# bliunlpr/Robust_e2e_gan

Measured on AMD Instinct MI355X. Metric: joint_train utterances/sec, higher is better.
Workload: dtype f32; 1 GPU; config4: joint_train.py full GAN+ASR step, B=32 per GPU, T=800, F=257->80, L=40, V=4233, enhancer 2xBLSTM-256, VGG+3xBLSTMP-512, loc-attention decoder 300, D basic ndf64, Adadelta; global_batch=32, per_rank_batch=32, parallelism=dp1, utterance_lengths=560..800 frames (mean 680 of T=800)

## Files before the change

robust_e2e_gan_amd/csrc/common.h:

```cpp
#pragma once
#include <hip/hip_runtime.h>
#include <mutex>
#include <stdint.h>
#include <stdlib.h>
#include <stdio.h>
#include <string.h>

#include "../../include/re2e.h"

typedef float f32x4 __attribute__((ext_vector_type(4)));
typedef float f32x16 __attribute__((ext_vector_type(16)));

#define RE2E_WAVE 64

void re2e_set_error(const char* fmt, ...);
bool re2e_stream_is_filler(hipStream_t stream);

#define RE2E_CHECK_ARG(cond, msg)                     \
  do {                                                \
    if (!(cond)) {                                    \
      re2e_set_error("%s: %s", __func__, msg);        \
      return RE2E_EINVAL;                             \
    }                                                 \
  } while (0)

#define RE2E_LAUNCH_CHECK()                                                        \
  do {                                                                             \
    hipError_t e__ = hipGetLastError();                                            \
    if (e__ != hipSuccess) {                                                       \
      re2e_set_error("%s: launch failed: %s", __func__, hipGetErrorString(e__));   \
      return RE2E_EHIP;                                                            \
    }                                                                              \
  } while (0)

#ifdef RE2E_EXPERIMENTS
static inline const char* exp_env(const char* name) { return getenv(name); }
#else
static inline const char* exp_env(const char*) { return nullptr; }
#endif

struct LdsLimit {
  std::mutex m;
  size_t set = 0;
  void ensure(const void* fn, size_t bytes) {
    std::lock_guard<std::mutex> g(m);
    if (bytes > set) {
      (void)hipFuncSetAttribute(fn, hipFuncAttributeMaxDynamicSharedMemorySize, (int)bytes);
      set = bytes;
    }
  }
};

static inline int cdiv(long a, long b) { return (int)((a + b - 1) / b); }

__device__ __forceinline__ float sigmoidf_(float x) { return 1.0f / (1.0f + __expf(-x)); }
__device__ __forceinline__ float tanhf_(float x) {
  float ax = fabsf(x);
  float e = __expf(-2.0f * ax);
  float t = (1.0f - e) / (1.0f + e);
  return copysignf(t, x);
}

__device__ __forceinline__ float wave_sum(float v) {
#pragma unroll
  for (int o = 32; o > 0; o >>= 1) v += __shfl_xor(v, o, 64);
  return v;
}
__device__ __forceinline__ float wave_max(float v) {
#pragma unroll
  for (int o = 32; o > 0; o >>= 1) v = fmaxf(v, __shfl_xor(v, o, 64));
  return v;
}

__device__ __forceinline__ float block_sum(float v, float* red) {
  v = wave_sum(v);
  int w = threadIdx.x >> 6, l = threadIdx.x & 63;
  __syncthreads();
  if (l == 0) red[w] = v;
  __syncthreads();
  int nw = (blockDim.x + 63) >> 6;
  float r = 0.f;
  for (int i = 0; i < nw; ++i) r += red[i];
  return r;
}
__device__ __forceinline__ float block_max(float v, float* red) {
  v = wave_max(v);
  int w = threadIdx.x >> 6, l = threadIdx.x & 63;
  __syncthreads();
  if (l == 0) red[w] = v;
  __syncthreads();
  int nw = (blockDim.x + 63) >> 6;
  float r = -3.0e38f;
  for (int i = 0; i < nw; ++i) r = fmaxf(r, red[i]);
  return r;
}

__device__ __forceinline__ float apply_act(float v, int act) {
  switch (act) {
    case RE2E_ACT_TANH: return tanhf_(v);
    case RE2E_ACT_RELU: return fmaxf(v, 0.f);
    case RE2E_ACT_LRELU: return v > 0.f ? v : 0.2f * v;
    case RE2E_ACT_SIGMOID: return sigmoidf_(v);
    default: return v;
  }
}

struct ConvGeom {
  const float* in; int NI, H, W, C; int PH, PW; int KH, KW; int SY, SX, DY, DX, OY0, OX0;
};

struct OutMap {
  float* out; long ldc; int remap; int PH, PW, OHF, OWF, osy, osx, ooy, oox;
  __device__ long off(int row) const {
    if (!remap) return (long)row * ldc;
    int j = row % PW; int t = row / PW; int i = t % PH; int n = t / PH;
    return (((long)n * OHF + i * osy + ooy) * OWF + j * osx + oox) * ldc;
  }
};

bool thin_conv_forward(const ConvGeom& g, const float* wg, int Cout, const OutMap& o, const float* bias, int act,
                       float beta, hipStream_t st);
int thin_wgrad_slabs(int C, int Cout, int KH, int KW, long P, long rows);
void thin_wgrad(const ConvGeom& g, const float* dout, int Cout, float* slabs, int nslab, hipStream_t st);

int gemm_kslices_tn(int M, int N, int K, int ns, const float* A, long lda, const float* B, long ldb, float* out, hipStream_t st, int nolog = 0);
int gemm_kslices(int M, int N, int K, int ns, const float* A, long lda, const float* B, long ldb, float* out, hipStream_t st, int nolog = 0);
size_t gemm_nt2_workspace_bytes(int M, int N, int K);
int gemm_nt2(int M, int N, int K, const float* A, long lda, const float* B, long ldb, float* C, long ldc, const float* bias, const float* bias2,
             int act, float beta, const float* mul, float* mask_out, const int* lens, int T, void* ws, size_t wsb, hipStream_t st,
             const int* rowmap = nullptr, int phys_rows = 0, int ident_rows = 0);
int gemm_nt2_kslices(int M, int N, int Ks, int ns, const float* A, long lda, const float* B, long ldb, float* out, hipStream_t st, int nolog);
size_t gemm_tn2_workspace_bytes(int M, int N, int K);
int gemm_tn2(int M, int N, int K, const float* A, long lda, const float* B, long ldb, float* C, long ldc, const float* bias, const float* bias2,
             int act, float beta, void* ws, size_t wsb, hipStream_t st);
int conv_nt2(const ConvGeom& g, int M, const float* wg, int Cout, float* out, long ldc, const float* bias, int act, float beta, int ncls,
             const int* cls_oy0, const int* cls_ox0, long cls_wstride, int remap, int OHF, int OWF, int osy, int osx, const int* ooy, const int* oox,
             hipStream_t st);
bool halo_conv3x3(const ConvGeom& g, const float* wg, int Cout, float* out, const float* bias, int act, float beta, const float* mask,
                  hipStream_t st, float* pool_out = nullptr, unsigned char* pool_idx = nullptr);
```

robust_e2e_gan_amd/csrc/core.hip:

```cpp
#include <stdarg.h>

#include <mutex>

#include "common.h"

static thread_local char g_err[512] = "";

void re2e_set_error(const char* fmt, ...) {
  va_list ap;
  va_start(ap, fmt);
  vsnprintf(g_err, sizeof(g_err), fmt, ap);
  va_end(ap);
}

extern "C" int re2e_version(void) { return RE2E_ABI_VERSION; }

extern "C" const char* re2e_last_error(void) { return g_err; }

extern "C" int re2e_device_ok(void) {
  hipDeviceProp_t prop;
  hipError_t e = hipGetDeviceProperties(&prop, 0);
  if (e != hipSuccess) {
    re2e_set_error("re2e_device_ok: %s", hipGetErrorString(e));
    return RE2E_EHIP;
  }
  return strncmp(prop.gcnArchName, "gfx950", 6) == 0 ? 1 : 0;
}

namespace {
std::mutex g_role_mu;
hipStream_t g_filler[64];
int g_nfiller = 0;
}

extern "C" int re2e_stream_role(hipStream_t stream, int role) {
  RE2E_CHECK_ARG(role == RE2E_STREAM_DEFAULT || role == RE2E_STREAM_FILLER, "role must be RE2E_STREAM_DEFAULT or RE2E_STREAM_FILLER");
  std::lock_guard<std::mutex> lock(g_role_mu);
  int at = -1;
  for (int i = 0; i < g_nfiller; ++i) if (g_filler[i] == stream) at = i;
  if (role == RE2E_STREAM_FILLER) {
    if (at >= 0) return RE2E_OK;
    if (g_nfiller == 64) { re2e_set_error("re2e_stream_role: more than 64 filler streams"); return RE2E_EINVAL; }
    g_filler[g_nfiller++] = stream;
  } else if (at >= 0) {
    g_filler[at] = g_filler[--g_nfiller];
  }
  return RE2E_OK;
}

bool re2e_stream_is_filler(hipStream_t stream) {
  static const bool ignore = exp_env("RE2E_IGNORE_STREAM_ROLE") != nullptr;
  if (ignore) return false;
  std::lock_guard<std::mutex> lock(g_role_mu);
  for (int i = 0; i < g_nfiller; ++i) if (g_filler[i] == stream) return true;
  return false;
}
```

robust_e2e_gan_amd/csrc/gemm_nt.hip:

```cpp
#include <stdlib.h>

#include "common.h"

namespace {

typedef unsigned u32x4_t __attribute__((ext_vector_type(4)));
constexpr unsigned OOB = 0x80000000u;

template <int WM_, int WN_, int TM_, int TN_, int BK_, int ST_, int WPS_>
struct NtCfg {
  static constexpr int WM = WM_, WN = WN_, TM = TM_, TN = TN_, BK = BK_, ST = ST_, WPS = WPS_;
  static constexpr int BM = WM_ * TM_ * 32, BN = WN_ * TN_ * 32;
  static constexpr int NW = WM_ * WN_, THREADS = NW * 64;
  static constexpr int RPP = 256 / BK_;
  static constexpr int CPR = BK_ / 4;
  static constexpr int RPL = 64 / BK_;
  static constexpr int PA = BM / RPP, PB = BN / RPP;
  static constexpr int NPW = (PA + PB) / NW;
  static constexpr int NPA = PA / NW;
  static constexpr int STAGE = (BM + BN) * BK_;
  static constexpr int NQ = BK_ / 8;
  static constexpr size_t LDS_BYTES = (size_t)ST_ * STAGE * 4;
  static_assert(PA % NW == 0 && PB % NW == 0, "pieces must divide over the waves per operand");
  static_assert(BK_ == 16 || BK_ == 32 || BK_ == 64, "BK");
// ... 320 lines not shown
            const unsigned soff = (unsigned)rowq * (unsigned)p.ldc * 4u;
            const unsigned vo = (rows_in || rowq + TM * 4 * lh < p.M) ? vlane : OOB;
            fTN v;
#pragma unroll
            for (int b = 0; b < TN; ++b) v[b] = apply_act(acc[a][b][r] + bq[b], act);
            if constexpr (TN == 4) {
              if (acc_old) v += __builtin_bit_cast(fTN, __builtin_amdgcn_raw_buffer_load_b128(rsC, vo, soff, 0));
              __builtin_amdgcn_raw_buffer_store_b128(__builtin_bit_cast(u32x4_t, v), rsC, vo, soff, 0);
            } else {
              typedef unsigned u32x2_t __attribute__((ext_vector_type(2)));
              if (acc_old) v += __builtin_bit_cast(fTN, __builtin_amdgcn_raw_buffer_load_b64(rsC, vo, soff, 0));
              __builtin_amdgcn_raw_buffer_store_b64(__builtin_bit_cast(u32x2_t, v), rsC, vo, soff, 0);
            }
          }
      }
    } else
    if (finish) {
      const __amdgpu_buffer_rsrc_t rsC = __builtin_amdgcn_make_buffer_rsrc(p.C + (MODE == 0 ? cls * p.batch_c : 0L), 0, 0x7FFFFFF0u, 0x00020000);
      const unsigned vlane = ((unsigned)(TNF ? TM * lr : lr) * (unsigned)p.ldc + 4u * (unsigned)lh) * 4u;
      const bool interior = !CONV && m0 + BM <= p.M && n0 + BN <= p.N;
      unsigned vrow[TM];
      const bool mapped = MODE == 0 && p.rowmap != nullptr && m0 + BM > p.ident_rows;
      if constexpr (MODE == 0) {
        if (mapped) {
#pragma unroll
          for (int a = 0; a < TM; ++a) {
            const int row = m0 + (wm * TM + a) * 32 + lr;
            vrow[a] = row < p.M ? (unsigned)(((long)p.rowmap[row] * p.ldc + 4 * lh) * 4) : OOB;
          }
        }
      }
      if constexpr (CONV) {
#pragma unroll
        for (int a = 0; a < TM; ++a) {
          const int row = m0 + (wm * TM + a) * 32 + lr;
          bool ok = row < p.M;
          long off = (long)row * p.ldc;
          if (p.remap) {
            const int px = row % p.cPW, t2 = row / p.cPW, py = t2 % p.cPH, n = t2 / p.cPH;
            const int oy = py * p.osy + p.ooy[cls], ox = px * p.osx + p.oox[cls];
            ok = ok && oy < p.OHF && ox < p.OWF;
            off = (((long)n * p.OHF + oy) * p.OWF + ox) * p.ldc;
          }
          vrow[a] = ok ? (unsigned)((off + 4 * lh) * 4) : OOB;
        }
      }
      const bool has_bias = p.bias != nullptr, has_bias2 = p.bias2 != nullptr;
      const int act = p.act;
      const bool acc_old = p.beta != 0.f;
#pragma unroll
      for (int b = 0; b < TN; ++b)
#pragma unroll
        for (int g = 0; g < 4; ++g) {
          const int colq = n0 + (wn * TN + b) * 32 + 8 * g;
          f32x4 bq = {0.f, 0.f, 0.f, 0.f};
          const bool col_ok = colq + 4 * lh < p.N;
          if (has_bias && col_ok) bq += *reinterpret_cast<const f32x4*>(p.bias + colq + 4 * lh);
          if (has_bias2 && col_ok) bq += *reinterpret_cast<const f32x4*>(p.bias2 + colq + 4 * lh);
#pragma unroll
          for (int a = 0; a < TM; ++a) {
            const int rowq = TNF ? m0 + wm * TM * 32 + a : m0 + (wm * TM + a) * 32;
            unsigned soff = ((unsigned)rowq * (unsigned)p.ldc + (unsigned)colq) * 4u;
            unsigned vo = (interior || (col_ok && rowq + (TNF ? TM * lr : lr) < p.M)) ? vlane : OOB;
            if constexpr (CONV) { soff = (unsigned)colq * 4u; vo = col_ok ? vrow[a] : OOB; }
            if constexpr (MODE == 0) { if (mapped) { soff = (unsigned)colq * 4u; vo = col_ok ? vrow[a] : OOB; } }
            f32x4 v = {acc[a][b][4 * g], acc[a][b][4 * g + 1], acc[a][b][4 * g + 2], acc[a][b][4 * g + 3]};
            v += bq;
            if (act == RE2E_ACT_TANH) {
#pragma unroll
              for (int e = 0; e < 4; ++e) v[e] = tanhf_(v[e]);
            } else if (act == RE2E_ACT_SIGMOID) {
#pragma unroll
              for (int e = 0; e < 4; ++e) v[e] = sigmoidf_(v[e]);
            } else if (act == RE2E_ACT_RELU) {
#pragma unroll
              for (int e = 0; e < 4; ++e) v[e] = v[e] < 0.f ? 0.f : v[e];
            } else if (act == RE2E_ACT_LRELU) {
#pragma unroll
              for (int e = 0; e < 4; ++e) v[e] = v[e] < 0.f ? 0.2f * v[e] : v[e];
            }
            if (acc_old) v += __builtin_bit_cast(f32x4, __builtin_amdgcn_raw_buffer_load_b128(rsC, vo, soff, 0));
            __builtin_amdgcn_raw_buffer_store_b128(__builtin_bit_cast(u32x4_t, v), rsC, vo, soff, 0);
          }
        }
    }
    u0 += ke - kb;
  }
}

using N256x128k32s3 = NtCfg<4, 2, 2, 2, 32, 3, 2>;
using N256x128k16s3 = NtCfg<4, 2, 2, 2, 16, 3, 4>;
using N128x128k32s2 = NtCfg<2, 2, 2, 2, 32, 2, 2>;
using N128x128k16s3 = NtCfg<2, 2, 2, 2, 16, 3, 3>;
using N128x64k16s4 = NtCfg<2, 2, 2, 1, 16, 4, 3>;
using N256x64k16s3 = NtCfg<4, 1, 2, 2, 16, 3, 2>;
using T128x128k16s3 = NtCfg<2, 2, 2, 2, 16, 3, 3>;

struct NtVariant { int id, bm, bn, bk, wg_per_cu; double tflops; };
const NtVariant VARIANTS[] = {{1, 256, 128, 32, 1, 130.0}, {3, 256, 128, 16, 2, 138.0}, {5, 128, 128, 32, 2, 130.0},
                              {6, 128, 128, 16, 3, 137.0}, {8, 128, 64, 16, 3, 136.0},  {9, 256, 64, 16, 2, 128.0}};

struct NtPlan { int variant; int wg_per_cu; int bm, bn, bk; int ntm, ntn, nkt, n_dp, g_sk; size_t bytes; double est; };

inline int num_cus() {
  static const int cus = [] { int dev = 0, n = 256; if (hipGetDevice(&dev) == hipSuccess) (void)hipDeviceGetAttribute(&n, hipDeviceAttributeMultiprocessorCount, dev); return n; }();
  return cus;
}

NtPlan nt2_plan_variant(const NtVariant& v, int M, int N, int K, int sk) {
  NtPlan pl;
  memset(&pl, 0, sizeof(pl));
  pl.variant = v.id; pl.bm = v.bm; pl.bn = v.bn; pl.bk = v.bk; pl.wg_per_cu = v.wg_per_cu;
  pl.ntm = cdiv(M, pl.bm); pl.ntn = cdiv(N, pl.bn); pl.nkt = cdiv(K, pl.bk);
  const long T = (long)pl.ntm * pl.ntn, cus = num_cus();
  const long R = T % cus;
  const double slab = (double)v.bm * v.bn * 4.0;
  const double t_tile = 2.0 * v.bm * v.bn * (double)K / (v.tflops * 1e12 / cus);
  const double t_over = 1.0e-6 + slab / 25e9;
  pl.n_dp = (int)T; pl.g_sk = 0;
  pl.est = (double)cdiv(T, cus) * (t_tile + t_over);
  if (sk && R != 0) {
    const long U = R * pl.nkt;
    long g = cus;
    if (T == R && v.bm * v.bn <= 128 * 256) { const char* e = exp_env("RE2E_NT2_TAILWG"); g = cus * (e ? atoi(e) : 1); }
    const long min_units = 128 / pl.bk;
    if (U / g < min_units) g = U / min_units;
    if (g >= 8) g &= ~7L;
    const double parts = (double)g / (double)R + 1.0;
    const double t_fix = (7e-6 + (double)g * slab / 2.4e12) * (T > R ? 0.7 : 1.0) + (parts > 3.0 ? (parts - 3.0) * slab / 80e9 : 0.0);
    const double est_sk = (double)(T / cus) * (t_tile + t_over) + (double)R / (double)g * t_tile / 0.93 + t_fix;
    if (g >= 2 && (sk == 2 || est_sk < pl.est)) { pl.n_dp = (int)(T - R); pl.g_sk = (int)g; pl.est = est_sk; }
  }
  pl.bytes = pl.g_sk ? (size_t)pl.g_sk * 2 * pl.bm * pl.bn * 4 : 0;
  return pl;
}

NtPlan nt2_plan(int M, int N, int K, bool filler, bool tn = false, int sk_override = -1) {
  int variant = 0, sk = 1;
  if (const char* e = exp_env(tn ? "RE2E_TN2" : "RE2E_NT2")) {
    if (e[0] == 'o') { NtPlan none; memset(&none, 0, sizeof(none)); return none; }
    variant = atoi(e);
    if (const char* c = strchr(e, ',')) sk = atoi(c + 1);
  }
  if (sk_override >= 0) sk = sk_override;
  NtPlan best;
  memset(&best, 0, sizeof(best));
  for (const NtVariant& v : VARIANTS) {
    if (variant ? v.id != variant : (tn ? v.id != 6 : (v.id == 1 || v.id == 5 || v.id == 9))) continue;
    if (!variant && filler && v.id == 3) continue;
    const NtPlan pl = nt2_plan_variant(v, M, N, K, sk);
    if (!best.variant || pl.est < best.est) best = pl;
  }
  return best;
}

constexpr int POOL_SLICES = 256, POOL_SLICE_INTS = 4096;
int* ticket_slice() {
  static std::mutex mu;
  static int* pool[16] = {nullptr};
  static unsigned next[16] = {0};
  int dev = 0;
  (void)hipGetDevice(&dev);
  if (dev < 0 || dev >= 16) return nullptr;
  std::lock_guard<std::mutex> g(mu);
  if (!pool[dev]) {
    if (hipMalloc(&pool[dev], (size_t)POOL_SLICES * POOL_SLICE_INTS * sizeof(int)) != hipSuccess) { pool[dev] = nullptr; return nullptr; }
    if (hipMemset(pool[dev], 0, (size_t)POOL_SLICES * POOL_SLICE_INTS * sizeof(int)) != hipSuccess) return nullptr;
  }
  return pool[dev] + (size_t)(next[dev]++ % POOL_SLICES) * POOL_SLICE_INTS;
}

template <class CF, int MODE>
void nt2_launch(const NtArgs& a, const NtPlan& pl, hipStream_t st) {
  static LdsLimit lim;
  size_t lds = CF::LDS_BYTES;
  int per_cu = pl.wg_per_cu;
  if (const char* e = exp_env("RE2E_NT2_MAXWG")) { const int m = atoi(e); if (m >= 1 && m < per_cu) per_cu = m; }
  const size_t want = (size_t)(160 * 1024) / (per_cu + 1) + 1024;
  if (lds < want) lds = want;
  lim.ensure(reinterpret_cast<const void*>(&gemm_nt2_kernel<CF, MODE>), lds);
  hipLaunchKernelGGL((gemm_nt2_kernel<CF, MODE>), dim3(pl.n_dp + pl.g_sk), dim3(CF::THREADS), lds, st, a);
}

}

size_t gemm_nt2_workspace_bytes(int M, int N, int K) {
  if (K % 4) return 0;
  const size_t a = nt2_plan(M, N, K, false).bytes, b = nt2_plan(M, N, K, true).bytes;
  return a > b ? a : b;
}

int conv_nt2(const ConvGeom& g, int M, const float* wg, int Cout, float* out, long ldc, const float* bias, int act, float beta, int ncls,
             const int* cls_oy0, const int* cls_ox0, long cls_wstride, int remap, int OHF, int OWF, int osy, int osx, const int* ooy, const int* oox,
             hipStream_t st) {
  if (const char* e = exp_env("RE2E_CONV_NT2")) { if (atoi(e) == 0) return 0; }
  const int K = g.KH * g.KW * g.C;
  if (g.C % 16 || Cout % 4 || g.KH * g.KW > 32 || g.KH * g.KW < 2 || ncls < 1 || ncls > 4) return 0;
  if ((reinterpret_cast<uintptr_t>(g.in) & 15) || (reinterpret_cast<uintptr_t>(wg) & 15) || (reinterpret_cast<uintptr_t>(out) & 15) || ldc % 4) return 0;
  if (bias && (reinterpret_cast<uintptr_t>(bias) & 15)) return 0;
  if (act == RE2E_ACT_SIGMOID_MASK_MUL || (long)M * ncls > 0x7FFFFFFFL || M < 256) return 0;
  const int ylo = g.DY < 0 ? (g.KH - 1) * g.DY : 0, xlo = g.DX < 0 ? (g.KW - 1) * g.DX : 0;
  int pady = 0, padx = 0;
  for (int c = 0; c < ncls; ++c) {
    const int oy = (cls_oy0 ? cls_oy0[c] : g.OY0) + ylo, ox = (cls_ox0 ? cls_ox0[c] : g.OX0) + xlo;
    if (-oy > pady) pady = -oy;
    if (-ox > padx) padx = -ox;
  }
  const long shift = ((long)pady * g.W + padx) * g.C * 4;
  const long in_bytes = (long)g.NI * g.H * g.W * g.C * 4;
  if (in_bytes + shift + (long)(g.KH * g.W + g.KW) * g.C * 4 * 4 >= 0x7FFFFFF0L) return 0;
  if ((long)ncls * Cout * K * 4 >= 0x7FFFFFF0L) return 0;
  NtPlan q = nt2_plan(M, Cout, K, re2e_stream_is_filler(st), false, 0);
  if (!q.variant || g.C % q.bk) return 0;
  q.n_dp = ncls * q.ntm * q.ntn; q.g_sk = 0;
  NtArgs a;
  memset(&a, 0, sizeof(a));
  a.A = reinterpret_cast<const float*>(reinterpret_cast<const char*>(g.in) - shift); a.B = wg; a.C = out;
  a.a_bytes = (unsigned)(in_bytes + shift); a.b_bytes = (unsigned)((long)ncls * Cout * K * 4);
  a.lda = 0; a.ldb = K; a.ldc = ldc; a.M = M; a.N = Cout; a.K = K;
  a.bias = bias; a.act = act; a.beta = beta;
  a.ntm = q.ntm; a.ntn = q.ntn; a.n_dp = q.n_dp; a.g_sk = q.g_sk; a.nkt = q.nkt;
  a.cH = g.H; a.cW = g.W; a.cC = g.C; a.cPH = g.PH; a.cPW = g.PW; a.cKH = g.KH; a.cKW = g.KW; a.cSY = g.SY; a.cSX = g.SX; a.cDY = g.DY; a.cDX = g.DX;
  a.ncls = ncls; a.cls_wstride = cls_wstride; a.remap = remap; a.OHF = OHF; a.OWF = OWF; a.osy = osy; a.osx = osx;
  for (int c = 0; c < 4; ++c) {
    a.cOY0[c] = cls_oy0 ? cls_oy0[c < ncls ? c : 0] : g.OY0; a.cOX0[c] = cls_ox0 ? cls_ox0[c < ncls ? c : 0] : g.OX0;
    a.ooy[c] = ooy ? ooy[c < ncls ? c : 0] : 0; a.oox[c] = oox ? oox[c < ncls ? c : 0] : 0;
  }
  a.a_shift = (unsigned)shift;
  static const bool log_calls = getenv("RE2E_IGEMM_LOG") != nullptr;
  if (log_calls)
    fprintf(stderr, "[igemm] A=ConvK B=DenseK tile=%dx%dx%d vec=1 M=%d N=%d K=%d splits=%d\n", q.bm, q.bn, q.bk, M * ncls, Cout, K, q.g_sk ? -q.g_sk : 1);
  if (exp_env("RE2E_NT2_LOG")) fprintf(stderr, "[conv2] %dx%dx%d cls %d variant %d tiles %ld dp %d sk %d\n", M, Cout, K, ncls, q.variant, (long)ncls * q.ntm * q.ntn, q.n_dp, q.g_sk);
  const NtPlan& pl2 = q;
  switch (pl2.variant) {
    case 1: nt2_launch<N256x128k32s3, 2>(a, pl2, st); break;
    case 3: nt2_launch<N256x128k16s3, 2>(a, pl2, st); break;
    case 5: nt2_launch<N128x128k32s2, 2>(a, pl2, st); break;
    case 6: nt2_launch<N128x128k16s3, 2>(a, pl2, st); break;
    case 8: nt2_launch<N128x64k16s4, 2>(a, pl2, st); break;
    case 9: nt2_launch<N256x64k16s3, 2>(a, pl2, st); break;
    default: return 0;
  }
  return 1;
}

int gemm_nt2_kslices(int M, int N, int Ks, int ns, const float* A, long lda, const float* B, long ldb, float* out, hipStream_t st, int nolog) {
  if (const char* e = exp_env("RE2E_NT2")) { if (e[0] == 'o') return 0; }
  if (Ks % 16 || lda % 4 || ldb % 4 || N % 4 || (reinterpret_cast<uintptr_t>(A) & 15) || (reinterpret_cast<uintptr_t>(B) & 15) || (reinterpret_cast<uintptr_t>(out) & 15)) return 0;
  const long K = (long)Ks * ns;
  if (((long)(M - 1) * lda + K) * 4 >= 0x7FFFFFF0L || ((long)(N - 1) * ldb + K) * 4 >= 0x7FFFFFF0L || (long)M * N * 4 >= 0x7FFFFFF0L || M < 256 || ns > 4096) return 0;
  NtPlan q = nt2_plan(M, N, Ks, re2e_stream_is_filler(st), false, 0);
  if (!q.variant) return 0;
  q.n_dp = ns * q.ntm * q.ntn; q.g_sk = 0;
  NtArgs a;
  memset(&a, 0, sizeof(a));
  a.A = A; a.B = B; a.C = out;
  a.a_bytes = (unsigned)(((long)(M - 1) * lda + K) * 4); a.b_bytes = (unsigned)(((long)(N - 1) * ldb + K) * 4);
  a.lda = (int)lda; a.ldb = (int)ldb; a.ldc = N; a.M = M; a.N = N; a.K = Ks;
  a.act = RE2E_ACT_NONE;
  a.ntm = q.ntm; a.ntn = q.ntn; a.n_dp = q.n_dp; a.g_sk = 0; a.nkt = q.nkt;
  a.ncls = ns; a.batch_k = Ks; a.batch_c = (long)M * N;
  static const bool log_calls = getenv("RE2E_IGEMM_LOG") != nullptr;
  if (log_calls && !nolog)
    fprintf(stderr, "[igemm] A=DenseK B=DenseK tile=%dx%dx%d vec=1 M=%d N=%d K=%ld splits=%d\n", q.bm, q.bn, q.bk, M, N, K, ns);
  switch (q.variant) {
    case 1: nt2_launch<N256x128k32s3, 0>(a, q, st); break;
    case 3: nt2_launch<N256x128k16s3, 0>(a, q, st); break;
    case 5: nt2_launch<N128x128k32s2, 0>(a, q, st); break;
    case 6: nt2_launch<N128x128k16s3, 0>(a, q, st); break;
    case 8: nt2_launch<N128x64k16s4, 0>(a, q, st); break;
    case 9: nt2_launch<N256x64k16s3, 0>(a, q, st); break;
    default: return 0;
  }
  return 1;
}

#ifdef RE2E_EXPERIMENTS
#include "experiments/gemm_tn2.hip"
#else
size_t gemm_tn2_workspace_bytes(int, int, int) { return 0; }
int gemm_tn2(int, int, int, const float*, long, const float*, long, float*, long, const float*, const float*, int, float, void*, size_t, hipStream_t) { return 0; }
#endif

int gemm_nt2(int M, int N, int K, const float* A, long lda, const float* B, long ldb, float* C, long ldc, const float* bias, const float* bias2,
             int act, float beta, const float* mul, float* mask_out, const int* lens, int T, void* ws, size_t wsb, hipStream_t st,
             const int* rowmap, int phys_rows, int ident_rows) {
  const int Mp = rowmap ? phys_rows : M;
  if (K % 4 || lda % 4 || ldb % 4 || (reinterpret_cast<uintptr_t>(A) & 15) || (reinterpret_cast<uintptr_t>(B) & 15)) return 0;
  if (((long)(Mp - 1) * lda + K) * 4 >= 0x7FFFFFF0L || ((long)(N - 1) * ldb + K) * 4 >= 0x7FFFFFF0L) return 0;
  if (M < 256 || Mp < M || act == RE2E_ACT_SIGMOID_MASK_MUL) return 0;
  (void)mul; (void)mask_out; (void)lens; (void)T;
  if (N % 4 || ldc % 4 || (reinterpret_cast<uintptr_t>(C) & 15) || ((long)(Mp - 1) * ldc + N) * 4 >= 0x7FFFFFF0L) return 0;
  if ((bias && (reinterpret_cast<uintptr_t>(bias) & 15)) || (bias2 && (reinterpret_cast<uintptr_t>(bias2) & 15))) return 0;
  const NtPlan pl = nt2_plan(M, N, K, re2e_stream_is_filler(st) || rowmap != nullptr);
  if (!pl.variant) return 0;
  NtArgs a;
  memset(&a, 0, sizeof(a));
  if (pl.g_sk) {
    if (!ws || wsb < pl.bytes || (long)pl.ntm * pl.ntn - pl.n_dp > POOL_SLICE_INTS) return 0;
    a.counters = ticket_slice();
    if (!a.counters) return 0;
    a.slabs = (float*)ws;
  }
  a.A = A; a.B = B; a.C = C;
  a.a_bytes = (unsigned)(((long)(Mp - 1) * lda + K) * 4); a.b_bytes = (unsigned)(((long)(N - 1) * ldb + K) * 4);
  a.lda = (int)lda; a.ldb = (int)ldb; a.ldc = ldc; a.M = M; a.N = N; a.K = K;
  a.bias = bias; a.bias2 = bias2; a.act = act; a.beta = beta;
  a.ntm = pl.ntm; a.ntn = pl.ntn; a.n_dp = pl.n_dp; a.g_sk = pl.g_sk; a.nkt = pl.nkt;
  a.rowmap = rowmap; a.ident_rows = rowmap ? ident_rows : 0;
  static const bool nomem = exp_env("RE2E_IGEMM_NOMEM") != nullptr;
  a.nomem = nomem ? 1 : 0;

  static const bool log_calls = getenv("RE2E_IGEMM_LOG") != nullptr;
  if (log_calls)
    fprintf(stderr, "[igemm] A=DenseK B=DenseK tile=%dx%dx%d vec=1 M=%d N=%d K=%d splits=%d\n", pl.bm, pl.bn, pl.bk, M, N, K, pl.g_sk ? -pl.g_sk : 1);
  if (exp_env("RE2E_NT2_LOG")) fprintf(stderr, "[nt2] %dx%dx%d variant %d tiles %ld dp %d sk %d est %.1f us\n", M, N, K, pl.variant, (long)pl.ntm * pl.ntn, pl.n_dp, pl.g_sk, pl.est * 1e6);
  switch (pl.variant) {
    case 1: nt2_launch<N256x128k32s3, 0>(a, pl, st); break;
    case 3: nt2_launch<N256x128k16s3, 0>(a, pl, st); break;
    case 5: nt2_launch<N128x128k32s2, 0>(a, pl, st); break;
    case 6: nt2_launch<N128x128k16s3, 0>(a, pl, st); break;
    case 8: nt2_launch<N128x64k16s4, 0>(a, pl, st); break;
// ... 48 lines not shown
```

robust_e2e_gan_amd/csrc/wino_wgrad.hip:

```cpp
#include <hip/hip_runtime.h>
#include "../../include/re2e.h"
#include "common.h"

namespace {
typedef float f32x16 __attribute__((ext_vector_type(16)));
typedef float f32x2 __attribute__((ext_vector_type(2)));
constexpr unsigned WW_OOB = 0x80000000u;
constexpr int WW_CB = 64, WW_OB = 32;

struct WwArgs {
  const float* x; const float* dy; float* slabs;
  int NI, H, W, C, Cout;
  int px, py, npatch, nsplit, ncb, nblk;
  unsigned x_bytes, dy_bytes;
  const int* row_lim;
  int flat;
  int dbg;
};

template <int TXW>
__global__ __launch_bounds__(256, 2) void wino_wgrad_kernel(WwArgs p) {
  constexpr int TYH = 32 / TXW, PW = 2 * TXW, PH = 2 * TYH;
  constexpr int XW = PW + 2, XH = PH + 2, XPIX = XW * XH;
  constexpr int XIT = (XPIX * 16 + 255) / 256, DIT = PW * PH * 8 / 256;
  extern __shared__ __attribute__((aligned(16))) float smem[];
  float* xs = smem;
  float* ds = smem + XPIX * WW_CB;
  const int tid = threadIdx.x, lane = tid & 63, lr = lane & 31, lh = lane >> 5;
  const int wid = __builtin_amdgcn_readfirstlane(tid >> 6);
  const int xk = blockIdx.x >> 3;
  const int blk = p.flat ? blockIdx.x % p.nblk : xk % p.nblk, split = p.flat ? blockIdx.x / p.nblk : (xk / p.nblk) * 8 + (blockIdx.x & 7);
  if (split >= p.nsplit) return;
  const int cb = blk % p.ncb, ob = blk / p.ncb;
  const int c0 = cb * WW_CB, o0 = ob * WW_OB;
  const __amdgpu_buffer_rsrc_t rsX = __builtin_amdgcn_make_buffer_rsrc(const_cast<float*>(p.x), 0, p.x_bytes, 0x00020000);
  const __amdgpu_buffer_rsrc_t rsD = __builtin_amdgcn_make_buffer_rsrc(const_cast<float*>(p.dy), 0, p.dy_bytes, 0x00020000);
  const int per = (p.npatch + p.nsplit - 1) / p.nsplit;
  const int pbeg = split * per, pend = min(p.npatch, pbeg + per);

  f32x4 xr[XIT], dr[DIT];
  auto load_patch = [&](int pi) {
    const int n = pi / (p.py * p.px), rem = pi - n * (p.py * p.px);
    const int pyi = rem / p.px, pxi = rem - pyi * p.px;
    const int y0 = pyi * PH, x0 = pxi * PW;
#pragma unroll
    for (int it = 0; it < XIT; ++it) {
      const int item = it * 256 + tid, pix = item >> 4, c4 = item & 15;
      const int yy = pix / XW, xx = pix - yy * XW, iy = y0 - 1 + yy, ix = x0 - 1 + xx;
      const bool ok = pix < XPIX && (unsigned)iy < (unsigned)p.H && (unsigned)ix < (unsigned)p.W;
      const unsigned off = (unsigned)((((n * p.H + iy) * p.W + ix) * p.C + c0 + c4 * 4) * 4);
      xr[it] = __builtin_bit_cast(f32x4, __builtin_amdgcn_raw_buffer_load_b128(rsX, ok ? off : WW_OOB, 0, 0));
    }
#pragma unroll
    for (int it = 0; it < DIT; ++it) {
      const int item = it * 256 + tid, pix = item >> 3, o4 = item & 7;
      const int yy = pix / PW, xx = pix - yy * PW, oy = y0 + yy, ox = x0 + xx;
      const bool ok = oy < p.H && ox < p.W;
      const unsigned off = (unsigned)((((n * p.H + oy) * p.W + ox) * p.Cout + o0 + o4 * 4) * 4);
      dr[it] = __builtin_bit_cast(f32x4, __builtin_amdgcn_raw_buffer_load_b128(rsD, ok ? off : WW_OOB, 0, 0));
    }
  };
  auto store_patch = [&]() {
#pragma unroll
    for (int it = 0; it < XIT; ++it) {
      const int item = it * 256 + tid;
      if (item < XPIX * 16) *reinterpret_cast<f32x4*>(xs + item * 4) = xr[it];
    }
#pragma unroll
    for (int it = 0; it < DIT; ++it) *reinterpret_cast<f32x4*>(ds + (it * 256 + tid) * 4) = dr[it];
  };

  const int rA = wid == 0 ? 0 : (wid == 2 ? 2 : 1), rB = wid == 3 ? 3 : (wid == 2 ? 1 : 2);
  const float sg = wid == 1 ? 1.f : -1.f;
  const float a0 = wid == 3 ? 0.f : 1.f, a1 = wid == 0 ? 0.f : (wid == 1 ? 1.f : -1.f);
  constexpr int HR = TYH / 2;
  const float* xA = xs + ((rA + 2 * HR * lh) * XW) * WW_CB + 2 * lr;
  const float* xB = xs + ((rB + 2 * HR * lh) * XW) * WW_CB + 2 * lr;
  const float* dB = ds + (2 * HR * lh * PW) * WW_OB + lr;

  f32x16 acc[4][2];
#pragma unroll
  for (int j = 0; j < 4; ++j)
#pragma unroll
    for (int ct = 0; ct < 2; ++ct)
#pragma unroll
      for (int r = 0; r < 16; ++r) acc[j][ct][r] = 0.f;

  for (int pi = pbeg; pi < pend; ++pi) {
    if (p.row_lim) {
      const int n = pi / (p.py * p.px), pyi = (pi - n * (p.py * p.px)) / p.px;
      if (pyi * PH >= p.row_lim[n]) continue;
    }
    load_patch(pi);
    store_patch();
    __syncthreads();
    f32x2 t[4], v[2][4];
    float m[2][4];
    auto prep = [&](const int s, f32x2 (&vv)[4], float (&mm)[4]) {
      const int tyl = s / TXW, txl = s % TXW;
#pragma unroll
      for (int j = 0; j < 4; ++j) {
        if (txl != 0 && j < 2) { t[j] = t[j + 2]; continue; }
        const f32x2 da = *reinterpret_cast<const f32x2*>(xA + ((2 * tyl) * XW + 2 * txl + j) * WW_CB);
        const f32x2 db = *reinterpret_cast<const f32x2*>(xB + ((2 * tyl) * XW + 2 * txl + j) * WW_CB);
        t[j] = da + sg * db;
      }
      vv[0] = t[0] - t[2]; vv[1] = t[1] + t[2]; vv[2] = t[2] - t[1]; vv[3] = t[1] - t[3];
      const float e00 = dB[((2 * tyl) * PW + 2 * txl) * WW_OB], e01 = dB[((2 * tyl) * PW + 2 * txl + 1) * WW_OB];
      const float e10 = dB[((2 * tyl + 1) * PW + 2 * txl) * WW_OB], e11 = dB[((2 * tyl + 1) * PW + 2 * txl + 1) * WW_OB];
      const float s0 = a0 * e00 + a1 * e10, s1 = a0 * e01 + a1 * e11;
      mm[0] = s0; mm[1] = s0 + s1; mm[2] = s0 - s1; mm[3] = -s1;
    };
    prep(0, v[0], m[0]);
#pragma unroll
    for (int s = 0; s < 16; ++s) {
      if (s + 1 < 16) prep(s + 1, v[(s + 1) & 1], m[(s + 1) & 1]);
#pragma unroll
      for (int j = 0; j < 4; ++j) {
        acc[j][0] = __builtin_amdgcn_mfma_f32_32x32x2f32(v[s & 1][j][0], m[s & 1][j], acc[j][0], 0, 0, 0);
        acc[j][1] = __builtin_amdgcn_mfma_f32_32x32x2f32(v[s & 1][j][1], m[s & 1][j], acc[j][1], 0, 0, 0);
      }
      if (s + 1 < 16) {
#pragma unroll
        for (int g = 0; g < 8; ++g) {
          __builtin_amdgcn_sched_group_barrier(0x008, 1, 0);
          __builtin_amdgcn_sched_group_barrier(0x100, 1, 0);
          __builtin_amdgcn_sched_group_barrier(0x002, 4, 0);
        }
      }
    }
    __syncthreads();
  }
  float* sl = p.slabs + ((long)split * 16 + 4 * wid) * p.C * p.Cout;
#pragma unroll
  for (int j = 0; j < 4; ++j)
#pragma unroll
    for (int ct = 0; ct < 2; ++ct)
#pragma unroll
      for (int r = 0; r < 16; ++r) {
        const int c = c0 + 2 * ((r & 3) + 8 * (r >> 2) + 4 * lh) + ct;
        sl[((long)j * p.C + c) * p.Cout + o0 + lr] = acc[j][ct][r];
      }
}

#ifdef RE2E_EXPERIMENTS
#include "experiments/wino_wgrad_dma.hip"
#endif

__global__ __launch_bounds__(1024) void wino_wgrad_reduce_kernel(const float* __restrict__ slabs, int nsplit, long tot, float* __restrict__ red) {
  __shared__ float part[16][64];
  const int e = threadIdx.x & 63, sl = threadIdx.x >> 6;
  const long i = (long)blockIdx.x * 64 + e;
  float s = 0.f;
  if (i < tot)
    for (int z = sl; z < nsplit; z += 16) s += slabs[(long)z * tot + i];
  part[sl][e] = s;
  __syncthreads();
  if (sl != 0 || i >= tot) return;
  s = 0.f;
#pragma unroll
  for (int q = 0; q < 16; ++q) s += part[q][e];
  red[i] = s;
}

__global__ __launch_bounds__(256) void wino_wgrad_final_kernel(const float* __restrict__ slabs, int nsplit, int C, int Cout, float* __restrict__ gw,
                                                               float beta) {
  const long i = (long)blockIdx.x * 256 + threadIdx.x;
  const long CO = (long)C * Cout;
  if (i >= CO) return;
  const int o = (int)(i % Cout), c = (int)(i / Cout);
  float u[4][4];
#pragma unroll
  for (int pos = 0; pos < 16; ++pos) u[pos >> 2][pos & 3] = 0.f;
  for (int s = 0; s < nsplit; ++s) {
    const float* sp = slabs + (long)s * 16 * CO + i;
#pragma unroll
    for (int pos = 0; pos < 16; ++pos) u[pos >> 2][pos & 3] += sp[pos * CO];
  }
  float t[3][4];
#pragma unroll
  for (int j = 0; j < 4; ++j) {
    t[0][j] = u[0][j] + 0.5f * (u[1][j] + u[2][j]);
    t[1][j] = 0.5f * (u[1][j] - u[2][j]);
    t[2][j] = 0.5f * (u[1][j] + u[2][j]) + u[3][j];
  }
  float* wp = gw + ((long)o * C + c) * 9;
#pragma unroll
  for (int a = 0; a < 3; ++a) {
    const float r0 = t[a][0] + 0.5f * (t[a][1] + t[a][2]), r1 = 0.5f * (t[a][1] - t[a][2]), r2 = 0.5f * (t[a][1] + t[a][2]) + t[a][3];
    if (beta != 0.f) { wp[a * 3] += r0; wp[a * 3 + 1] += r1; wp[a * 3 + 2] += r2; }
    else { wp[a * 3] = r0; wp[a * 3 + 1] = r1; wp[a * 3 + 2] = r2; }
  }
}

struct WwPlan { bool wide; int px, py, npatch, nsplit, ncb, nblk; size_t bytes; };
WwPlan ww_plan(int NI, int H, int W, int C, int Cout) {
  WwPlan q;
  const long pad_w = (long)cdiv(H, 8) * 8 * cdiv(W, 16) * 16, pad_n = (long)cdiv(H, 16) * 16 * cdiv(W, 8) * 8;
  q.wide = pad_w <= pad_n;
  q.px = cdiv(W, q.wide ? 16 : 8); q.py = cdiv(H, q.wide ? 8 : 16);
  q.npatch = NI * q.py * q.px;
  q.ncb = C / WW_CB; q.nblk = q.ncb * (Cout / WW_OB);
  int s = cdiv(1536, q.nblk);
  if (s > q.npatch / 8) s = q.npatch / 8;
  if (s < 1) s = 1;
  q.nsplit = s;
  q.bytes = (size_t)(s + 1) * 16 * C * Cout * sizeof(float);
  return q;
}

template <int TXW>
void launch_ww(const WwArgs& a, hipStream_t st) {
  constexpr int PW = 2 * TXW, PH = 64 / TXW;
#ifdef RE2E_EXPERIMENTS
  static const bool dma = exp_env("RE2E_WW_DMA") && atoi(exp_env("RE2E_WW_DMA")) == 1;
  if (dma) {
    constexpr size_t lds2 = (size_t)2 * (192 * WW_CB + PW * PH * WW_OB) * sizeof(float);
    static LdsLimit lim2;
    lim2.ensure(reinterpret_cast<const void*>(&wino_wgrad_dma_kernel<TXW>), lds2);
    hipLaunchKernelGGL((wino_wgrad_dma_kernel<TXW>), dim3((unsigned)(cdiv(a.nsplit, 8) * 8 * a.nblk)), dim3(256), lds2, st, a);
    return;
  }
#endif
  constexpr size_t lds = (size_t)((PW + 2) * (PH + 2) * WW_CB + PW * PH * WW_OB) * sizeof(float);
  static LdsLimit lim;
  lim.ensure(reinterpret_cast<const void*>(&wino_wgrad_kernel<TXW>), lds);
  hipLaunchKernelGGL((wino_wgrad_kernel<TXW>), dim3((unsigned)(cdiv(a.nsplit, 8) * 8 * a.nblk)), dim3(256), lds, st, a);
}
}

extern "C" size_t re2e_conv3x3_wino_wgrad_workspace_bytes(int NI, int H, int W, int C, int Cout) {
  if (NI <= 0 || H <= 0 || W <= 0 || C <= 0 || Cout <= 0 || C % WW_CB || Cout % WW_OB) return 0;
  return ww_plan(NI, H, W, C, Cout).bytes;
}

static int ww_impl(const float* in, int NI, int H, int W, int C, const float* dout, int Cout, float* gw, float beta, const int* row_lim, void* workspace,
                   size_t workspace_bytes, hipStream_t stream) {
  RE2E_CHECK_ARG(in && dout && gw && workspace, "null operand");
  RE2E_CHECK_ARG(NI > 0 && H > 0 && W > 0 && C > 0 && Cout > 0, "bad geometry");
  RE2E_CHECK_ARG(beta == 0.f || beta == 1.f, "beta must be 0 or 1");
  if (C % WW_CB || Cout % WW_OB) { re2e_set_error("re2e_conv3x3_wino_wgrad: C must be a multiple of 64 and Cout of 32 (got %d, %d)", C, Cout); return RE2E_EUNSUPPORTED; }
  const long x_bytes = (long)NI * H * W * C * 4, dy_bytes = (long)NI * H * W * Cout * 4;
  if (x_bytes >= 0x7FFFFF00L || dy_bytes >= 0x7FFFFF00L) { re2e_set_error("re2e_conv3x3_wino_wgrad: tensors must be < 2 GiB"); return RE2E_EUNSUPPORTED; }
  RE2E_CHECK_ARG((reinterpret_cast<uintptr_t>(in) & 15) == 0 && (reinterpret_cast<uintptr_t>(dout) & 15) == 0, "in / dout must be 16-byte aligned");
  const WwPlan q = ww_plan(NI, H, W, C, Cout);
  RE2E_CHECK_ARG(workspace_bytes >= q.bytes, "workspace too small (re2e_conv3x3_wino_wgrad_workspace_bytes)");
  WwArgs a;
  a.x = in; a.dy = dout; a.slabs = static_cast<float*>(workspace);
  a.NI = NI; a.H = H; a.W = W; a.C = C; a.Cout = Cout;
  a.px = q.px; a.py = q.py; a.npatch = q.npatch; a.nsplit = q.nsplit; a.ncb = q.ncb; a.nblk = q.nblk;
  a.x_bytes = (unsigned)x_bytes; a.dy_bytes = (unsigned)dy_bytes;
  a.row_lim = row_lim;
  a.dbg = exp_env("RE2E_WW_DBG") ? atoi(exp_env("RE2E_WW_DBG")) : 0;
  a.flat = exp_env("RE2E_WW_FLAT") ? atoi(exp_env("RE2E_WW_FLAT")) : 0;
  static const bool log_calls = getenv("RE2E_IGEMM_LOG") != nullptr;
  if (log_calls)
    fprintf(stderr, "[igemm] A=WinoW B=DenseM tile=64x32x2 vec=1 M=%d N=%d K=%ld splits=%d\n", 9 * C, Cout, (long)NI * H * W, q.nsplit);
  if (q.wide) launch_ww<8>(a, stream); else launch_ww<4>(a, stream);
  const long tot = 16L * C * Cout;
  float* red = a.slabs + (long)q.nsplit * tot;
  hipLaunchKernelGGL(wino_wgrad_reduce_kernel, dim3((unsigned)cdiv(tot, 64)), dim3(1024), 0, stream, a.slabs, q.nsplit, tot, red);
  hipLaunchKernelGGL(wino_wgrad_final_kernel, dim3((unsigned)cdiv((long)C * Cout, 256)), dim3(256), 0, stream, red, 1, C, Cout, gw, beta);
  RE2E_LAUNCH_CHECK();
  return RE2E_OK;
}

extern "C" int re2e_conv3x3_wino_wgrad(const float* in, int NI, int H, int W, int C, const float* dout, int Cout, float* gw, float beta, void* workspace,
                                       size_t workspace_bytes, hipStream_t stream) {
  return ww_impl(in, NI, H, W, C, dout, Cout, gw, beta, nullptr, workspace, workspace_bytes, stream);
}

extern "C" int re2e_conv3x3_wino_wgrad_rows(const float* in, int NI, int H, int W, int C, const float* dout, int Cout, float* gw, float beta,
                                            const int* row_lim, void* workspace, size_t workspace_bytes, hipStream_t stream) {
  RE2E_CHECK_ARG(row_lim, "null row limits");
  return ww_impl(in, NI, H, W, C, dout, Cout, gw, beta, row_lim, workspace, workspace_bytes, stream);
}
```

Measured before the change: 684.6 utterances/s.

## Fuse Winograd wgrad split reduction into main kernel via atomic ticket tree

The Winograd weight-gradient kernel now reduces its split-K partials itself. Each block writes its accumulator slab, takes an atomic ticket per quad-tree node, and the last arriver sums its children, so the root applies the inverse Winograd transform and writes gw directly. This removes the separate reduce and final kernel launches and their slab traffic. The split count is now derived from a resident-block target of 512 instead of 1536, patches are strided rather than contiguous per split, and a global ticket pool is shared with the GEMM code. The cost is that reductions run serially in the tail blocks, and correctness depends on the counter reset and on memory visibility between blocks.

```diff
diff --git a/robust_e2e_gan_amd/csrc/common.h b/robust_e2e_gan_amd/csrc/common.h
--- a/robust_e2e_gan_amd/csrc/common.h
+++ b/robust_e2e_gan_amd/csrc/common.h
@@ -50,6 +50,9 @@
     }
   }
 };
+
+constexpr int POOL_SLICE_INTS = 4096;
+int* ticket_slice();
 
 static inline int cdiv(long a, long b) { return (int)((a + b - 1) / b); }
 
diff --git a/robust_e2e_gan_amd/csrc/core.hip b/robust_e2e_gan_amd/csrc/core.hip
--- a/robust_e2e_gan_amd/csrc/core.hip
+++ b/robust_e2e_gan_amd/csrc/core.hip
@@ -55,3 +55,19 @@
   for (int i = 0; i < g_nfiller; ++i) if (g_filler[i] == stream) return true;
   return false;
 }
+
+int* ticket_slice() {
+  constexpr int POOL_SLICES = 256;
+  static std::mutex mu;
+  static int* pool[16] = {nullptr};
+  static unsigned next[16] = {0};
+  int dev = 0;
+  (void)hipGetDevice(&dev);
+  if (dev < 0 || dev >= 16) return nullptr;
+  std::lock_guard<std::mutex> g(mu);
+  if (!pool[dev]) {
+    if (hipMalloc(&pool[dev], (size_t)POOL_SLICES * POOL_SLICE_INTS * sizeof(int)) != hipSuccess) { pool[dev] = nullptr; return nullptr; }
+    if (hipMemset(pool[dev], 0, (size_t)POOL_SLICES * POOL_SLICE_INTS * sizeof(int)) != hipSuccess) return nullptr;
+  }
+  return pool[dev] + (size_t)(next[dev]++ % POOL_SLICES) * POOL_SLICE_INTS;
+}
diff --git a/robust_e2e_gan_amd/csrc/gemm_nt.hip b/robust_e2e_gan_amd/csrc/gemm_nt.hip
--- a/robust_e2e_gan_amd/csrc/gemm_nt.hip
+++ b/robust_e2e_gan_amd/csrc/gemm_nt.hip
@@ -496,22 +496,6 @@
     if (!best.variant || pl.est < best.est) best = pl;
   }
   return best;
-}
-
-constexpr int POOL_SLICES = 256, POOL_SLICE_INTS = 4096;
-int* ticket_slice() {
-  static std::mutex mu;
-  static int* pool[16] = {nullptr};
-  static unsigned next[16] = {0};
-  int dev = 0;
-  (void)hipGetDevice(&dev);
-  if (dev < 0 || dev >= 16) return nullptr;
-  std::lock_guard<std::mutex> g(mu);
-  if (!pool[dev]) {
-    if (hipMalloc(&pool[dev], (size_t)POOL_SLICES * POOL_SLICE_INTS * sizeof(int)) != hipSuccess) { pool[dev] = nullptr; return nullptr; }
-    if (hipMemset(pool[dev], 0, (size_t)POOL_SLICES * POOL_SLICE_INTS * sizeof(int)) != hipSuccess) return nullptr;
-  }
-  return pool[dev] + (size_t)(next[dev]++ % POOL_SLICES) * POOL_SLICE_INTS;
 }
 
 template <class CF, int MODE>
diff --git a/robust_e2e_gan_amd/csrc/wino_wgrad.hip b/robust_e2e_gan_amd/csrc/wino_wgrad.hip
--- a/robust_e2e_gan_amd/csrc/wino_wgrad.hip
+++ b/robust_e2e_gan_amd/csrc/wino_wgrad.hip
@@ -5,13 +5,19 @@
 namespace {
 typedef float f32x16 __attribute__((ext_vector_type(16)));
 typedef float f32x2 __attribute__((ext_vector_type(2)));
+typedef unsigned u32x4_t __attribute__((ext_vector_type(4)));
 constexpr unsigned WW_OOB = 0x80000000u;
 constexpr int WW_CB = 64, WW_OB = 32;
+constexpr int WW_BLK = 16 * WW_CB * WW_OB;
+constexpr int WW_RESIDENT = 512;
 
 struct WwArgs {
   const float* x; const float* dy; float* slabs;
+  float* gw; float beta;
+  int* counters;
   int NI, H, W, C, Cout;
   int px, py, npatch, nsplit, ncb, nblk;
+  int nlev, cpb;
   unsigned x_bytes, dy_bytes;
   const int* row_lim;
   int flat;
@@ -35,8 +41,6 @@
   const int c0 = cb * WW_CB, o0 = ob * WW_OB;
   const __amdgpu_buffer_rsrc_t rsX = __builtin_amdgcn_make_buffer_rsrc(const_cast<float*>(p.x), 0, p.x_bytes, 0x00020000);
   const __amdgpu_buffer_rsrc_t rsD = __builtin_amdgcn_make_buffer_rsrc(const_cast<float*>(p.dy), 0, p.dy_bytes, 0x00020000);
-  const int per = (p.npatch + p.nsplit - 1) / p.nsplit;
-  const int pbeg = split * per, pend = min(p.npatch, pbeg + per);
 
   f32x4 xr[XIT], dr[DIT];
   auto load_patch = [&](int pi) {
@@ -86,7 +90,7 @@
 #pragma unroll
       for (int r = 0; r < 16; ++r) acc[j][ct][r] = 0.f;
 
-  for (int pi = pbeg; pi < pend; ++pi) {
+  for (int pi = split; pi < p.npatch; pi += p.nsplit) {
     if (p.row_lim) {
       const int n = pi / (p.py * p.px), pyi = (pi - n * (p.py * p.px)) / p.px;
       if (pyi * PH >= p.row_lim[n]) continue;
@@ -131,21 +135,98 @@
     }
     __syncthreads();
   }
-  float* sl = p.slabs + ((long)split * 16 + 4 * wid) * p.C * p.Cout;
+
+  const __amdgpu_buffer_rsrc_t rsS = __builtin_amdgcn_make_buffer_rsrc(p.slabs, 0, 0x7FFFFFF0u, 0x00020000);
+  const unsigned lane_off = (unsigned)tid * 16u;
+  auto slab_off = [&](int s) { return (unsigned)(((long)s * p.nblk + blk) * WW_BLK * 4); };
+  int node = split, lev = 0, lev_base = 0;
+  while (lev < p.nlev) {
+    const int span = 1 << (2 * lev);
+    const unsigned so = slab_off(node * span) + lane_off;
+#pragma unroll
+    for (int j = 0; j < 4; ++j)
+#pragma unroll
+      for (int ct = 0; ct < 2; ++ct)
+#pragma unroll
+        for (int g = 0; g < 4; ++g) {
+          const f32x4 v = {acc[j][ct][4 * g], acc[j][ct][4 * g + 1], acc[j][ct][4 * g + 2], acc[j][ct][4 * g + 3]};
+          __builtin_amdgcn_raw_buffer_store_b128(__builtin_bit_cast(u32x4_t, v), rsS, so + (unsigned)(((j * 2 + ct) * 4 + g) * 256 * 16), 0, 16);
+        }
+    asm volatile("s_waitcnt vmcnt(0)" ::: "memory");
+    __syncthreads();
+    const int parent = node >> 2, pfirst = parent * span * 4;
+    const int nchild = min(4, (p.nsplit - pfirst + span - 1) / span);
+    int* const ctr = p.counters + blk * p.cpb + lev_base + parent;
+    if (tid == 0) smem[0] = __int_as_float(__hip_atomic_fetch_add(ctr, 1, __ATOMIC_RELAXED, __HIP_MEMORY_SCOPE_AGENT));
+    __syncthreads();
+    const int old = __float_as_int(smem[0]);
+    __syncthreads();
+    if (old != nchild - 1) return;
+    if (tid == 0) *ctr = 0;
+#pragma unroll
+    for (int j = 0; j < 4; ++j)
+#pragma unroll
+      for (int ct = 0; ct < 2; ++ct)
+#pragma unroll
+        for (int r = 0; r < 16; ++r) acc[j][ct][r] = 0.f;
+    for (int k = 0; k < nchild; ++k) {
+      const unsigned co = slab_off(pfirst + k * span) + lane_off;
+#pragma unroll
+      for (int j = 0; j < 4; ++j)
+#pragma unroll
+        for (int ct = 0; ct < 2; ++ct) {
+          f32x4 v[4];
+#pragma unroll
+          for (int g = 0; g < 4; ++g)
+            v[g] = __builtin_bit_cast(f32x4, __builtin_amdgcn_raw_buffer_load_b128(rsS, co + (unsigned)(((j * 2 + ct) * 4 + g) * 256 * 16), 0, 16));
+#pragma unroll
+          for (int g = 0; g < 4; ++g)
+#pragma unroll
+            for (int e = 0; e < 4; ++e) acc[j][ct][4 * g + e] += v[g][e];
+        }
+    }
+    lev_base += (p.nsplit + span * 4 - 1) / (span * 4);
+    node = parent;
+    ++lev;
+  }
+
+  const unsigned ro = (unsigned)(((long)p.nsplit * p.nblk + blk) * WW_BLK * 4);
 #pragma unroll
   for (int j = 0; j < 4; ++j)
 #pragma unroll
     for (int ct = 0; ct < 2; ++ct)
 #pragma unroll
       for (int r = 0; r < 16; ++r) {
-        const int c = c0 + 2 * ((r & 3) + 8 * (r >> 2) + 4 * lh) + ct;
-        sl[((long)j * p.C + c) * p.Cout + o0 + lr] = acc[j][ct][r];
+        const int c = 2 * ((r & 3) + 8 * (r >> 2) + 4 * lh) + ct;
+        __builtin_amdgcn_raw_buffer_store_b32(__float_as_uint(acc[j][ct][r]), rsS, ro + (unsigned)((((4 * wid + j) * WW_OB + lr) * WW_CB + c) * 4), 0, 16);
       }
+  asm volatile("s_waitcnt vmcnt(0)" ::: "memory");
+  __syncthreads();
+  for (int e = tid; e < WW_CB * WW_OB; e += 256) {
+    const int c = e % WW_CB, o = e / WW_CB;
+    float u[4][4];
+#pragma unroll
+    for (int pos = 0; pos < 16; ++pos)
+      u[pos >> 2][pos & 3] = __uint_as_float(__builtin_amdgcn_raw_buffer_load_b32(rsS, ro + (unsigned)((pos * WW_OB * WW_CB + e) * 4), 0, 16));
+    float t[3][4];
+#pragma unroll
+    for (int j = 0; j < 4; ++j) {
+      t[0][j] = u[0][j] + 0.5f * (u[1][j] + u[2][j]);
+      t[1][j] = 0.5f * (u[1][j] - u[2][j]);
+      t[2][j] = 0.5f * (u[1][j] + u[2][j]) + u[3][j];
+    }
+    float* wp = p.gw + ((long)(o0 + o) * p.C + c0 + c) * 9;
+#pragma unroll
+    for (int a = 0; a < 3; ++a) {
+      const float r0 = t[a][0] + 0.5f * (t[a][1] + t[a][2]), r1 = 0.5f * (t[a][1] - t[a][2]), r2 = 0.5f * (t[a][1] + t[a][2]) + t[a][3];
+      if (p.beta != 0.f) { wp[a * 3] += r0; wp[a * 3 + 1] += r1; wp[a * 3 + 2] += r2; }
+      else { wp[a * 3] = r0; wp[a * 3 + 1] = r1; wp[a * 3 + 2] = r2; }
+    }
+  }
 }
 
 #ifdef RE2E_EXPERIMENTS
 #include "experiments/wino_wgrad_dma.hip"
-#endif
 
 __global__ __launch_bounds__(1024) void wino_wgrad_reduce_kernel(const float* __restrict__ slabs, int nsplit, long tot, float* __restrict__ red) {
   __shared__ float part[16][64];
@@ -192,8 +273,9 @@
     else { wp[a * 3] = r0; wp[a * 3 + 1] = r1; wp[a * 3 + 2] = r2; }
   }
 }
-
-struct WwPlan { bool wide; int px, py, npatch, nsplit, ncb, nblk; size_t bytes; };
+#endif
+
+struct WwPlan { bool wide; int px, py, npatch, nsplit, ncb, nblk, nlev, cpb; size_t bytes; };
 WwPlan ww_plan(int NI, int H, int W, int C, int Cout) {
   WwPlan q;
   const long pad_w = (long)cdiv(H, 8) * 8 * cdiv(W, 16) * 16, pad_n = (long)cdiv(H, 16) * 16 * cdiv(W, 8) * 8;
@@ -201,11 +283,14 @@
   q.px = cdiv(W, q.wide ? 16 : 8); q.py = cdiv(H, q.wide ? 8 : 16);
   q.npatch = NI * q.py * q.px;
   q.ncb = C / WW_CB; q.nblk = q.ncb * (Cout / WW_OB);
-  int s = cdiv(1536, q.nblk);
+  static const int resident = exp_env("RE2E_WW_RESIDENT") ? atoi(exp_env("RE2E_WW_RESIDENT")) : WW_RESIDENT;
+  int s = resident / q.nblk;
   if (s > q.npatch / 8) s = q.npatch / 8;
   if (s < 1) s = 1;
   q.nsplit = s;
-  q.bytes = (size_t)(s + 1) * 16 * C * Cout * sizeof(float);
+  q.nlev = 0; q.cpb = 0;
+  for (long span = 1; span < s; span *= 4) { ++q.nlev; q.cpb += cdiv(s, span * 4); }
+  q.bytes = (size_t)(s + 1) * q.nblk * WW_BLK * sizeof(float);
   return q;
 }
 
@@ -219,6 +304,10 @@
     static LdsLimit lim2;
     lim2.ensure(reinterpret_cast<const void*>(&wino_wgrad_dma_kernel<TXW>), lds2);
     hipLaunchKernelGGL((wino_wgrad_dma_kernel<TXW>), dim3((unsigned)(cdiv(a.nsplit, 8) * 8 * a.nblk)), dim3(256), lds2, st, a);
+    const long tot = 16L * a.C * a.Cout;
+    float* red = a.slabs + (long)a.nsplit * tot;
+    hipLaunchKernelGGL(wino_wgrad_reduce_kernel, dim3((unsigned)cdiv(tot, 64)), dim3(1024), 0, st, a.slabs, a.nsplit, tot, red);
+    hipLaunchKernelGGL(wino_wgrad_final_kernel, dim3((unsigned)cdiv((long)a.C * a.Cout, 256)), dim3(256), 0, st, red, 1, a.C, a.Cout, a.gw, a.beta);
     return;
   }
 #endif
@@ -245,10 +334,18 @@
   RE2E_CHECK_ARG((reinterpret_cast<uintptr_t>(in) & 15) == 0 && (reinterpret_cast<uintptr_t>(dout) & 15) == 0, "in / dout must be 16-byte aligned");
   const WwPlan q = ww_plan(NI, H, W, C, Cout);
   RE2E_CHECK_ARG(workspace_bytes >= q.bytes, "workspace too small (re2e_conv3x3_wino_wgrad_workspace_bytes)");
+  if (q.bytes >= 0x7FFFFF00UL || (long)q.nblk * q.cpb > POOL_SLICE_INTS) {
+    re2e_set_error("re2e_conv3x3_wino_wgrad: %d x %d channels are more than one launch reduces", C, Cout);
+    return RE2E_EUNSUPPORTED;
+  }
   WwArgs a;
   a.x = in; a.dy = dout; a.slabs = static_cast<float*>(workspace);
+  a.gw = gw; a.beta = beta;
+  a.counters = ticket_slice();
+  if (!a.counters) { re2e_set_error("re2e_conv3x3_wino_wgrad: no ticket pool"); return RE2E_EHIP; }
   a.NI = NI; a.H = H; a.W = W; a.C = C; a.Cout = Cout;
   a.px = q.px; a.py = q.py; a.npatch = q.npatch; a.nsplit = q.nsplit; a.ncb = q.ncb; a.nblk = q.nblk;
+  a.nlev = q.nlev; a.cpb = q.cpb;
   a.x_bytes = (unsigned)x_bytes; a.dy_bytes = (unsigned)dy_bytes;
   a.row_lim = row_lim;
   a.dbg = exp_env("RE2E_WW_DBG") ? atoi(exp_env("RE2E_WW_DBG")) : 0;
@@ -257,10 +354,6 @@
   if (log_calls)
     fprintf(stderr, "[igemm] A=WinoW B=DenseM tile=64x32x2 vec=1 M=%d N=%d K=%ld splits=%d\n", 9 * C, Cout, (long)NI * H * W, q.nsplit);
   if (q.wide) launch_ww<8>(a, stream); else launch_ww<4>(a, stream);
-  const long tot = 16L * C * Cout;
-  float* red = a.slabs + (long)q.nsplit * tot;
-  hipLaunchKernelGGL(wino_wgrad_reduce_kernel, dim3((unsigned)cdiv(tot, 64)), dim3(1024), 0, stream, a.slabs, q.nsplit, tot, red);
-  hipLaunchKernelGGL(wino_wgrad_final_kernel, dim3((unsigned)cdiv((long)C * Cout, 256)), dim3(256), 0, stream, red, 1, C, Cout, gw, beta);
   RE2E_LAUNCH_CHECK();
   return RE2E_OK;
 }
```

Result: no change. 684.7 utterances/s, median of 4 (+0.0%).
